# iesl/anncur

Hardware: AMD Instinct MI355X
Metric: queries/sec + Top-k-Recall@100 vs exact, CUR-256 on QxI score matrix (higher is better)
Workload: dtype bf16; 1 GPU; cfg2: Q=10000/GPU x I=100000 bf16 score matrix, 256 anchor items, 512 anchor queries, k=100, k_retvr=100; step = gather C_q + fused S_hat/top-k + exact top-k scan + overlap/recall; Q_per_gpu=10000, I=100000, anchors=256, anchor_queries=512, k=100, k_retvr=100

## Files before the change

### anncur_amd/csrc/common.hpp

```cpp
#pragma once
#include <hip/hip_runtime.h>
#include <stdint.h>
#include <stdarg.h>
#include <stdio.h>
#include "anncur_hip.h"

void anncur_set_error(const char *fmt, ...);
constexpr int LADDER_LEVELS = 8;
int anncur_internal_kth_value(const float *G, int64_t Q, int n, int64_t ldg, int k, float *out, int64_t out_stride, hipStream_t st, int coarse = 0,
							  float *ladder = nullptr, int k2 = 1, float *tau2 = nullptr);
int anncur_internal_approx_error_acc(const void *X, int x_dtype, int64_t ldx, const void *Et, int e_dtype, int64_t lde, const void *Aex, int a_dtype,
									 int64_t lda, int64_t Q, int64_t I, int64_t K, float *err_sq, float *norm_sq, void *stream);

int anncur_ensure_dyn_lds(const void *fn, int bytes);
int anncur_num_cu();
int anncur_event_pool(hipEvent_t **out, int n);
int anncur_internal_scan_rows_in_flight(int dtype);

#define ANNCUR_REQUIRE(cond, code, ...)                 \
	do {                                                \
		if (!(cond)) {                                  \
			anncur_set_error(__VA_ARGS__);              \
			return (code);                              \
		}                                               \
	} while (0)

#define ANNCUR_HIP_OK(expr)                                                              \
	do {                                                                                 \
		hipError_t e__ = (expr);                                                         \
		if (e__ != hipSuccess) {                                                         \
			anncur_set_error("%s failed: %s (%s:%d)", #expr, hipGetErrorString(e__), __FILE__, __LINE__); \
			return ANNCUR_E_HIP;                                                         \
		}                                                                                \
// ... 81 lines not shown
```

### anncur_amd/csrc/score16.hpp

```cpp
#pragma once

typedef __attribute__((ext_vector_type(4))) float f32x4;

template <int KP, int NW = 4>
struct Fused16Cfg {
	static constexpr int WAVES = NW;
	static constexpr int KS32 = KP / 32;
	static constexpr int K = KP / 16;
	static constexpr int CPR = KP / 8;
	static constexpr int TILE_BYTES = TILE_I * KP * 2;
	static constexpr int QCAP = 1024;
	static constexpr int DRAIN_AT = 192;
	static constexpr int QUEUE_OFF = 2 * TILE_BYTES;
	static constexpr int CNT_OFF = QUEUE_OFF + NW * QCAP * 8;
	static constexpr int TICKET_OFF = CNT_OFF + NW * 64 * 4;
	static constexpr int PIECES = TILE_BYTES / 1024 / NW;
	static_assert(PIECES >= 1, "a tile holds at least one 1 KB piece per wave");
	static constexpr int LVL_OFF = TICKET_OFF + 16;
	static constexpr int LCNT_OFF = LVL_OFF + NW * 64 * 4 * LADDER_LEVELS;
	static constexpr int JCUR_OFF = LCNT_OFF + NW * 64 * 16;
	static constexpr int LDS_BYTES = JCUR_OFF + NW * 64 * 4;
	static_assert(NW != 4 || LDS_BYTES <= 80 * 1024, "two workgroups per CU");
	static_assert(LADDER_LEVELS == 8, "two 128-bit reads per query; eight 16-bit fields in four counter words");
	static constexpr int BQ = 64 * NW;
// ... 158 lines not shown
		lds_wait_frag(ring[g % AR], after < DIST ? after : DIST);
		const bf16x8 a = __builtin_bit_cast(bf16x8, ring[g % AR]);
		const int s = g % K, ks = s >> 1, ih = s & 1;
		if (g < K) {
			accA[ih][0] = __builtin_amdgcn_mfma_f32_16x16x32_bf16(a, xb[0][ks], accA[ih][0], 0, 0, 0);
			accA[ih][1] = __builtin_amdgcn_mfma_f32_16x16x32_bf16(a, xb[1][ks], accA[ih][1], 0, 0, 0);
#pragma unroll
			for (int e = (g == 1 ? 0 : g) * EPS; e < (g == 0 ? 0 : g + 1) * EPS; ++e) F16_ELEM(accP, e, 2, tau_prev, item0_prev);
		} else {
			accB[ih][0] = __builtin_amdgcn_mfma_f32_16x16x32_bf16(a, xb[2][ks], accB[ih][0], 0, 0, 0);
			accB[ih][1] = __builtin_amdgcn_mfma_f32_16x16x32_bf16(a, xb[3][ks], accB[ih][1], 0, 0, 0);
#pragma unroll
			for (int e = (g - K == 1 ? 0 : g - K) * EPS; e < (g == K ? 0 : g - K + 1) * EPS; ++e) F16_ELEM(accA, e, 0, tau, item0);
		}
	}
#pragma unroll
	for (int ih = 0; ih < 2; ++ih)
#pragma unroll
		for (int q = 0; q < 2; ++q) accP[ih][q] = accB[ih][q];
#undef F16_READ
}

#define S16_SLICED (p.sliced)
template <int KP, int NW = 4>
__global__ __launch_bounds__(64 * NW, 2) void score16_kernel(const FusedParams p) {
	using C = Fused16Cfg<KP, NW>;
	constexpr int K = C::K, KS32 = C::KS32, CPR = C::CPR;
	extern __shared__ __attribute__((aligned(16))) unsigned char smem[];
	const int tid = threadIdx.x, lane = tid & 63, wave = tid >> 6;
	const int c16 = lane & 15, g4 = lane >> 4;
	const int wid = xcd_remap(blockIdx.x, p.n_wg);
	const int n_rb = (int)((p.Q + C::BQ - 1) / C::BQ);
	const int split = wid / n_rb, rb = wid - split * n_rb;

	bf16x8 xb[4][KS32];
	int64_t qv[4];
#pragma unroll
	for (int t = 0; t < 4; ++t) {
		qv[t] = (int64_t)rb * C::BQ + wave * 64 + 16 * t + c16;
		const bool ok = qv[t] < p.Q;
		const u32x4 *src = reinterpret_cast<const u32x4 *>(p.X + (ok ? qv[t] : 0) * p.ldx) + g4;
#pragma unroll
		for (int s = 0; s < KS32; ++s) {
			const u32x4 zero = {0u, 0u, 0u, 0u};
			const u32x4 w = ok ? src[4 * s] : zero;
			xb[t][s] = __builtin_bit_cast(bf16x8, w);
// ... 44 lines not shown
	const bool dyn = p.chunk_tiles > 0;
	uint32_t ticket_slot = lds_addr(smem + C::TICKET_OFF);
	uint32_t *const ctr_rb = p.chunk_ctr + (S16_SLICED ? (size_t)rb * N_SLICES : (size_t)rb);
	int slice = S16_SLICED ? xcc_id() : 0, tried = 0;
	if (dyn) {
		if (tid == 0) {
			uint32_t c0, c1;
			if (S16_SLICED) {
				c0 = slice_resolve(atomicAdd(ctr_rb + slice, 1u), ctr_rb, p.n_chunks, p.chunks_per_slice, slice, tried);
				c1 = c0 < (uint32_t)p.n_chunks ? slice_resolve(atomicAdd(ctr_rb + slice, 1u), ctr_rb, p.n_chunks, p.chunks_per_slice, slice, tried) : (uint32_t)p.n_chunks;
			} else {
				c0 = atomicAdd(ctr_rb, 2u); c1 = c0 + 1u;
			}
			if (p.chunk_owner) {
				if (c0 < (uint32_t)p.n_chunks) p.chunk_owner[(int64_t)rb * p.n_chunks + c0] = (uint8_t)split;
				if (c1 < (uint32_t)p.n_chunks) p.chunk_owner[(int64_t)rb * p.n_chunks + c1] = (uint8_t)split;
			}
			lds_write_u32(ticket_slot + 8u, c0);
			lds_write_u32(ticket_slot + 12u, c1);
			__builtin_amdgcn_s_waitcnt(0xC07F);
		}
		__syncthreads();
		const uint32_t c = lds_load_u32_uniform(ticket_slot + 8u), c1 = lds_load_u32_uniform(ticket_slot + 12u);
		t_cur = c < (uint32_t)p.n_chunks ? p.tile_begin + (int)c * p.chunk_tiles : -1;
		t_cend = min(t_cur + p.chunk_tiles, p.tile_end);
		t_next_chunk = c1 < (uint32_t)p.n_chunks ? p.tile_begin + (int)c1 * p.chunk_tiles : -1;
	}
	uint32_t dma_off[C::PIECES];
#pragma unroll
	for (int i = 0; i < C::PIECES; ++i) {
		const int pch = (wave_u * C::PIECES + i) * 64 + lane;
		const int row = pch / CPR, cs = pch % CPR;
		dma_off[i] = (uint32_t)(row * CPR + swz<CPR>(row, cs)) * 16u;
	}
	auto tile_dma_w = [&](int tile, uint32_t lds_buf) {
		const unsigned char *src = reinterpret_cast<const unsigned char *>(p.Et) + (int64_t)tile * C::TILE_BYTES;
#if defined(__HIP_DEVICE_COMPILE__)
#pragma unroll
		for (int i = 0; i < C::PIECES; ++i) {
			const uint32_t m0v = lds_buf + (uint32_t)(wave_u * C::PIECES + i) * 1024u;
			asm volatile("s_mov_b32 m0, %0\n\ts_nop 0\n\tglobal_load_lds_dwordx4 %1, %2" ::"s"(m0v), "v"(dma_off[i]), "s"(src) : "memory", "m0");
		}
#endif
	};
	if (t_cur >= 0) tile_dma_w(t_cur, lds_base);
	__builtin_amdgcn_s_waitcnt(0x0F70);
	__syncthreads();

	f32x4 accP[2][2];
// ... 11 lines not shown
	float tau_hi[2] = {tau[2], tau[3]};
#define R16_DRAIN_CHECK(J) do { if (fill >= w.base + C::DRAIN_AT * 8u) wq_drain<true>(w, fill); } while (0)
#define LADDER_STEP()                                                                                                           \
	do {                                                                                                                        \
		if (p.ladder_on) {                                                                                                      \
			const uint32_t ll_ = opaque_u32((uint32_t)lane);    \
			if (lad_pending) {                                                                                                  \
				ladder_refresh(lcnt_land + ll_ * 16u, w.lvl + ll_ * 32u, w.jcur + ll_ * 4u, p.ladder_k, (int)(ll_ & 15u), tau);     \
				tau_hi[0] = tau[2]; tau_hi[1] = tau[3];                                                                         \
				tau_prev[0] = fmaxf(tau_prev[0], tau[2]); tau_prev[1] = fmaxf(tau_prev[1], tau[3]);                             \
				lad_pending = false;                                                                                            \
			}                                                                                                                   \
			if ((++lad_tick & p.ladder_mask) == 0u) {                                                                           \
				ladder_fetch(w.lcnt, lcnt_land, (int)ll_);                                                                      \
				lad_pending = true;                                                                                             \
			}                                                                                                                   \
		}                                                                                                                       \
	} while (0)
#define STAGGER16_STEP(CUR)                                                                                                     \
	do {                                                                                                                        \
		const int J = t_cur;                                                                                                    \
		if (ticket_pending) {                                                                                                   \
			const uint32_t c = lds_load_u32_uniform(ticket_slot);                                                               \
			t_next_chunk = c < (uint32_t)p.n_chunks ? p.tile_begin + (int)c * p.chunk_tiles : -1;                               \
			ticket_pending = false;                                                                                             \
			ticket_slot ^= 4u;                                                                                                  \
		}                                                                                                                       \
		int nx = J + 1;                                                                                                         \
		bool crossed = false;                                                                                                   \
		if (nx >= t_cend) { nx = t_next_chunk; crossed = dyn && nx >= 0; }                                                      \
		if (nx >= 0) tile_dma_w(nx, lds_base + ((CUR) ^ 1) * C::TILE_BYTES);                                                    \
		uint32_t ticket = 0;                                                                                                    \
		if (crossed && tid == 0) ticket_draw(ticket, ctr_rb + slice);                                                           \
		LADDER_STEP();                                                                                                          \
		R16_DRAIN_CHECK(J);                                                                                                     \
		const uint32_t item0 = ((uint32_t)J * TILE_I + 4 * g4) | lane_code;                                                     \
		stagger16_tile<KP, CUR>(aoff, xb, accP, tau, tau_prev, item0, item0_prev, w, fill);                                        \
		tau_prev[0] = tau_hi[0]; tau_prev[1] = tau_hi[1]; item0_prev = item0;                                                   \
		ticket_wait(ticket);                                                                                                    \
		if (crossed) {                                                                                                          \
			if (tid == 0) {                                                                                                     \
				if (S16_SLICED) ticket = slice_resolve(ticket, ctr_rb, p.n_chunks, p.chunks_per_slice, slice, tried);             \
				lds_write_u32(ticket_slot, ticket);                                                                             \
				if (p.chunk_owner && ticket < (uint32_t)p.n_chunks) p.chunk_owner[(int64_t)rb * p.n_chunks + ticket] = (uint8_t)split; \
				__builtin_amdgcn_s_waitcnt(0xC07F);                                                                             \
			}                                                                                                                   \
			ticket_pending = true;                                                                                              \
			t_cend = min(nx + p.chunk_tiles, p.tile_end);                                                                       \
		}                                                                                                                       \
		__syncthreads();                                                                                                        \
		t_cur = nx;                                                                                                             \
	} while (0)
	ANNCUR_PAD_HERE();
	while (t_cur >= 0) {
		STAGGER16_STEP(0);
		if (t_cur < 0) break;
		STAGGER16_STEP(1);
	}
#undef STAGGER16_STEP
#undef LADDER_STEP
	wq_drain<true>(w, fill);
#define F16_LAST(e)                                                                                                             \
	filter16_one(accP[(e) >> 3][((e) >> 2) & 1][(e) & 3],                                                                       \
				 (uint32_t)((((e) >> 3) * 16 + ((e) & 3)) | ((uint32_t)(2 + (((e) >> 2) & 1)) << (WQ_ITEM_BITS + 4))),         \
				 tau_prev[((e) >> 2) & 1], item0_prev, w, fill)
	F16_LAST(0); F16_LAST(1); F16_LAST(2); F16_LAST(3); F16_LAST(4); F16_LAST(5); F16_LAST(6); F16_LAST(7);
	F16_LAST(8); F16_LAST(9); F16_LAST(10); F16_LAST(11); F16_LAST(12); F16_LAST(13); F16_LAST(14); F16_LAST(15);
#undef F16_LAST
#undef F16_ELEM
	wq_drain<true>(w, fill);
	if (p.ladder_on) {
		const int le = (int)opaque_u32((uint32_t)lane);
// ... 25 lines not shown
```

### anncur_amd/csrc/score_fused.hip

```cpp
#include <stdlib.h>
#include <math.h>
#include <type_traits>
#ifdef ANNCUR_PLACEMENT_PAD
#define ANNCUR_PAD_HERE() asm volatile(".rept %0\n\ts_nop 0\n\t.endr" ::"n"(ANNCUR_PLACEMENT_PAD) : "memory")
#else
#define ANNCUR_PAD_HERE() do { } while (0)
#endif
#include "select.hpp"
#include "wave_select.hpp"
#include "select_stream.hpp"

using namespace anncur;

namespace {

typedef __attribute__((ext_vector_type(8))) __bf16 bf16x8;
typedef __attribute__((ext_vector_type(16))) float f32x16;
typedef __attribute__((ext_vector_type(4))) unsigned int u32x4;

constexpr int TILE_I = 32;
constexpr int CHUNK_TILES = 4;

template <int KP, int QTV = ((KP <= 256) ? 2 : 1)>
struct FusedCfg {
// ... 18 lines not shown
}

struct FusedParams {
	const uint16_t *X; int64_t ldx;
	const uint16_t *Et;
	int64_t Q, I;
	int n_tiles, n_full_tiles;
	int S, tiles_per_split;
	int tile_begin, tile_end;
	int tile_step;
	int carry;
	int n_st, S0, st_per_split;
	int sample_leading;
	float *gmax; int n_groups;
	const float *tau; int tau_stride;
	uint2 *cand; uint32_t *seg_cnt; int capg;
	int nseg;
	int flush_tiles;
	int n_wg;
	int chunk_tiles, n_chunks;
	uint32_t *chunk_ctr;
	uint8_t *chunk_owner;
	int sliced, chunks_per_slice;
	int ladder_on; uint32_t ladder_k, ladder_mask;
	const float *ladder; uint32_t *ladder_cnt; float *tau_final;
	uint32_t *nfb;
	uint32_t zero_bytes;
};

__device__ __forceinline__ int xcd_remap(int b, int n) {
	const int q = n >> 3, r = n & 7, x = b & 7, l = b >> 3;
	return (x < r ? x * (q + 1) : r * (q + 1) + (x - r) * q) + l;
}

__device__ __forceinline__ void zero_ws_header(const FusedParams &p) {
	typedef __attribute__((ext_vector_type(4))) unsigned int zvec;
	zvec *const dst = reinterpret_cast<zvec *>(p.nfb);
	const uint32_t n = p.zero_bytes >> 4;
	for (uint32_t i = blockIdx.x * blockDim.x + threadIdx.x; i < n; i += gridDim.x * blockDim.x) dst[i] = (zvec){0u, 0u, 0u, 0u};
}


template <int KP>
__device__ __forceinline__ void tile_dma(const uint16_t *__restrict__ Et, int tile, unsigned char *buf, int wave, int lane) {
	constexpr int CPR = FusedCfg<KP>::CPR;
	constexpr int PER_WAVE = FusedCfg<KP>::TILE_BYTES / 1024 / 4;
	const unsigned char *src = reinterpret_cast<const unsigned char *>(Et + (int64_t)tile * TILE_I * KP);
#pragma unroll
	for (int i = 0; i < PER_WAVE; ++i) {
		const int piece = wave * PER_WAVE + i;
		const int pch = piece * 64 + lane;
// ... 812 lines not shown
		 \
		 \
		asm volatile("" ::: "memory");                                                                                          \
		__builtin_amdgcn_s_barrier();                                                                                           \
		asm volatile("" ::: "memory");                                                                                          \
	} while (0)
	for (int j = j_begin; j < j_end; j += 2) {
		ERR_STEP(0, j);
		if (j + 1 < j_end) ERR_STEP(1, j + 1);
	}
#undef ERR_STEP
#pragma unroll
	for (int t = 0; t < QT; ++t)
		if (qv[t] < p.Q) {
			atomicAdd(&err_sq[qv[t]], se[t]);
			atomicAdd(&norm_sq[qv[t]], sn[t]);
		}
}

#include "score_evalf.hpp"

struct SweepStages {
	int n, begin[3], end[3], tps[3], stride;
	int chunk, bq, n_chunks[3];
	const uint8_t *owner[3];
};

template <int KMAX>
__global__ __launch_bounds__(SEL_THREADS) void select_candidates_kernel(
	const uint2 *__restrict__ cand, const uint32_t *__restrict__ seg_cnt, int nseg, int S, SweepStages stg, int capg,
	const uint16_t *__restrict__ X, int64_t ldx, const uint16_t *__restrict__ Et, int64_t I, int KP, uint32_t k,
	float *__restrict__ out_val, int32_t *__restrict__ out_idx, uint32_t *__restrict__ n_fallback,
	const int32_t *__restrict__ hard_list, const uint32_t *__restrict__ hard_cnt, const float *__restrict__ tau_in, int tau_stride,
	const int32_t *__restrict__ remap) {
	extern __shared__ __attribute__((aligned(16))) unsigned char smem[];
	const SelState s = sel_carve<KMAX>(smem);
	float *xq = reinterpret_cast<float *>(smem + SelCfg<KMAX>::LDS_BYTES);
	uint32_t *bad = reinterpret_cast<uint32_t *>(xq + KP);
	const int tid = threadIdx.x, lane = tid & 63, wave = tid >> 6;
	auto score_of = [&](int64_t i) {
		float v = 0.f;
		const uint4 *er = reinterpret_cast<const uint4 *>(Et + i * KP);
		for (int c = 0; c < KP / 8; ++c) {
			const uint4 w = er[c];
			const uint32_t ww[4] = {w.x, w.y, w.z, w.w};
#pragma unroll
			for (int d = 0; d < 4; ++d) {
// ... 38 lines not shown
			for (uint32_t e0 = 0; e0 < maxc; e0 += WAVE) {
				const uint32_t e = e0 + lane;
				const bool in = e < c;
				const uint2 ce = in ? sp_ptr[e] : make_uint2(0, 0);
				sel_offer(s, in, __uint_as_float(ce.x), ce.y, tau, tau_key);
				sel_maybe_compact<KMAX>(s, k, tau, tau_key);
			}
		}
	}
	if (repair || full) {
		if (tid == 0) atomicAdd(n_fallback, 1u);
		for (int c = tid; c < KP; c += SEL_THREADS) xq[c] = bf16_bits_to_f32(X[q * ldx + c]);
		__syncthreads();
	}
	if (repair) {
		for (int sp = 0; sp < S; ++sp) {
			if (!((bad[sp >> 5] >> (sp & 31)) & 1u)) continue;
			for (int g = 0; g < stg.n; ++g) {
				if (stg.chunk > 0) {
					const uint8_t *own = stg.owner[g] + (q / stg.bq) * (int64_t)stg.n_chunks[g];
					int it = 0;
					for (int c = 0; c < stg.n_chunks[g]; ++c) {
						if (own[c] != (uint8_t)sp) continue;
						const int64_t i_beg = (int64_t)(stg.begin[g] + c * stg.chunk) * TILE_I;
						const int64_t i_end = (int64_t)min(stg.begin[g] + (c + 1) * stg.chunk, stg.end[g]) * TILE_I;
						for (int64_t i0 = i_beg; i0 < i_end; i0 += SEL_THREADS, ++it) {
							const int64_t i = i0 + tid;
							const bool in = i < i_end && i < I;
							const float v = in ? score_of(i) : 0.f;
							sel_offer(s, in, v, (uint32_t)i, tau, tau_key);
							if ((it & 15) == 15) sel_maybe_compact<KMAX>(s, k, tau, tau_key);
						}
					}
					sel_maybe_compact<KMAX>(s, k, tau, tau_key);
					continue;
				}
				if (stg.stride > 1) {
					int it = 0;
					for (int tb = stg.begin[g] + sp; tb < stg.end[g]; tb += 8 * stg.stride, ++it) {
						const int tile = tb + (tid >> 5) * stg.stride;
						const int64_t i = (int64_t)tile * TILE_I + (tid & 31);
						const bool in = tile < stg.end[g] && i < I;
						const float v = in ? score_of(i) : 0.f;
						sel_offer(s, in, v, (uint32_t)i, tau, tau_key);
						if ((it & 15) == 15) sel_maybe_compact<KMAX>(s, k, tau, tau_key);
					}
					sel_maybe_compact<KMAX>(s, k, tau, tau_key);
					continue;
// ... 138 lines not shown
	wsel_finish<0, 4, WqCfg<KW>::E, true>(w, k, out_val + q * (int64_t)k, out_idx + q * (int64_t)k, remap);
}

}
namespace {
#include "score_wide.hpp"
}
namespace {

struct FusedPlan {
	bool ok;
	bool wide;
	int QT, BQ, n_rb, n_tiles, n_full, S, tiles_per_split, group, n_st, S0, st_per_split, n_groups, capg, kmax, flush_tiles;
	int n_stages, stage_end[3], stage_tps[3], stage_flush[3], stage_pred[3];
	int leading;
	int lg;
	int nseg;
	bool body16;
	bool bodyef;
	bool bodyq16;
	int chunk;
	bool ladder;
	int ladder_k2;
	size_t off_lcnt, off_lvl, off_tau2;
	size_t off_gmax, off_tval, off_tidx, off_segcnt, off_cand, off_tau, off_hard, off_ctr, off_owner, total;
};

int num_cu() { return anncur_num_cu(); }

size_t align256(size_t x) { return (x + 255) & ~(size_t)255; }
int next_pow2(int x) { int p = 1; while (p < x) p <<= 1; return p; }

void plan_stages(FusedPlan &P, int64_t Q, int k, double exp_hits, bool staged, double fmin, int unit_items) {
	double frac[3] = {1.0, 1.0, 1.0};
	P.n_stages = 1;
	if (staged) {
		const double H0 = exp_hits, c_hit = 2.4e-11 * (double)Q;
		const double c_stage = k <= WSEL_K ? 25e-6 + 3e-9 * (double)Q : (k <= WQ_K2 ? 25e-6 + 1.2e-8 * (double)Q : 25e-6 + 1.4e-11 * (double)Q * 0.3 * H0);
		auto later = [&](double f) { const double h = 1.2 * k / f; return h < H0 ? h : H0; };
		double best = H0 * c_hit;
		static const double grid[] = {0.02, 0.03, 0.04, 0.06, 0.08, 0.10, 0.12, 0.15, 0.18, 0.22, 0.26, 0.30, 0.35, 0.40, 0.50};
		const int ng = (int)(sizeof(grid) / sizeof(grid[0]));
		for (int i = 0; i < ng; ++i) {
			const double f1 = grid[i];
			if (f1 < fmin) continue;
			const double c2 = (f1 * H0 + (1 - f1) * later(f1)) * c_hit + c_stage;
// ... 106 lines not shown
	if (S > 255) S = P.chunk > 0 ? 255 : (S > 256 ? 256 : S);
	if (S > P.n_tiles) S = P.n_tiles;
	P.tiles_per_split = (P.n_tiles + S - 1) / S;
	P.S = (P.n_tiles + P.tiles_per_split - 1) / P.tiles_per_split;
	constexpr int64_t LADDER_WAVE_SLACK = (int64_t)(LADDER_PERIOD + 2) * TILE_I + Fused16Cfg<256>::DRAIN_AT;
	const bool ladder_fits = I < 65536 || (int64_t)k + (int64_t)P.S * LADDER_WAVE_SLACK <= 32768;
	const bool ladder_possible = !no_ladder && ticketed && P.n_groups <= 4096 && ladder_fits;
	P.body16 = can16 && !mfma32 && !evalf && (mfma16 || k <= (ladder_possible ? BODY16_MAX_K_LADDER : BODY16_MAX_K));
	plan_prepass_splits(P, slots);
	P.lg = (P.body16 || P.bodyq16 || P.bodyef) ? 1 : 2;
	const double exp_hits = plan_segments(P, k, leading);
	const double per_lane_tile = exp_hits / ((double)P.n_tiles * 2.0);
	int ft = (int)(0.35 / (per_lane_tile > 1e-9 ? per_lane_tile : 1e-9));
	P.flush_tiles = ft < 1 ? 1 : (ft > 8 ? 8 : ft);
	P.ladder = P.body16 && ladder_possible;
	{
		double r = (double)k * ((double)P.n_st * TILE_I / (double)I) * (leading ? 2.0 : 1.25);
		int k2 = (int)(r + 0.5);
		if (k2 > k / 2) k2 = k / 2;
		if (k2 < 3) k2 = 3;
		if (k2 > k) k2 = k;
		P.ladder_k2 = k2;
	}
	plan_stages(P, Q, k, exp_hits, !P.ladder && (k <= WQ_K2 ? P.nseg <= WAVE : true) && P.n_tiles >= 24 * P.S, 4.0 * P.S / P.n_tiles, TILE_I);
	plan_workspace(P, Q, k, (size_t)P.n_rb * 3 * 4 * N_SLICES, (size_t)3 * P.n_rb * (size_t)(P.n_tiles / (P.chunk > 0 ? P.chunk : P.n_tiles) + 2));
	return P;
}

int launch_tau_refine(const uint2 *cand, const uint32_t *seg_cnt, int nseg, int capg, int64_t Q, int k, int kmax, float *tau, int tau_stride,
					  int prefilter, hipStream_t st) {
	int rc;
	if (k <= WQ_K2 && nseg <= WAVE) {
		if (k <= WSEL_K) {
			constexpr int lds = 4 * WaveSelLayout<WqCfg<128>::CAP>::BYTES;
			if ((rc = anncur_ensure_dyn_lds((const void *)select_wave_kernel<true, 128>, lds)) != ANNCUR_OK) return rc;
			hipLaunchKernelGGL((select_wave_kernel<true, 128>), dim3((unsigned)ceil_div64(Q, 4)), dim3(256), lds, st, cand, seg_cnt, nseg, capg, Q,
							   (uint32_t)k, (float *)nullptr, (int32_t *)nullptr, (uint32_t *)nullptr, (int32_t *)nullptr, tau, tau_stride, prefilter, (const int32_t *)nullptr);
		} else {
			constexpr int lds = 4 * StreamSelLayout::BYTES;
			hipLaunchKernelGGL((select_stream_kernel<true, 2>), dim3((unsigned)ceil_div64(Q, 4)), dim3(256), lds, st, cand, seg_cnt, nseg, capg, Q,
							   (uint32_t)k, (float *)nullptr, (int32_t *)nullptr, (uint32_t *)nullptr, (int32_t *)nullptr, tau, tau_stride, prefilter, (const int32_t *)nullptr);
		}
	} else {
#define LAUNCH_TAU(KM)                                                                                                        \
		do {                                                                                                                  \
			if ((rc = anncur_ensure_dyn_lds((const void *)tau_block_kernel<KM>, (int)SelCfg<KM>::LDS_BYTES)) != ANNCUR_OK) return rc; \
// ... 37 lines not shown
			constexpr int lds = 4 * StreamSelLayout::BYTES;                                                                       \
			hipLaunchKernelGGL((select_stream_kernel<false, EE>), dim3((unsigned)ceil_div64(Q, 4)), dim3(256), lds, st, cand, seg_cnt, P.nseg, P.capg, Q, \
							   (uint32_t)k, out_val, out_idx, hc, hl, const_cast<float *>(tau), tau_stride, (P.n_stages > 1 || P.ladder) ? 1 : 0, remap); \
		} while (0)
		if (k <= WSEL_K) LAUNCH_WSEL(128);
		else if (k <= 256) LAUNCH_SSEL(4);
		else if (k <= 512) LAUNCH_SSEL(8);
		else LAUNCH_SSEL(16);
#undef LAUNCH_SSEL
#undef LAUNCH_WSEL
		ANNCUR_LAUNCH_OK();
		hard_list = hl; hard_cnt = hc;
		sel_grid = (unsigned)(Q < 1024 ? Q : 1024);
	}
	if (P.kmax == 128) LAUNCH_SELECT(128); else if (P.kmax == 512) LAUNCH_SELECT(512); else LAUNCH_SELECT(2048);
#undef LAUNCH_SELECT
	ANNCUR_LAUNCH_OK();
	return ANNCUR_OK;
}

int launch_threshold(const FusedPlan &P, const float *gmax, int64_t Q, int k, unsigned char *ws, const float *&tau, int &tau_stride, hipStream_t st) {
	if (P.n_groups <= 4096) {
		float *t = (float *)(ws + P.off_tau);
		const int rc = P.ladder ? anncur_internal_kth_value(gmax, Q, P.n_groups, P.n_groups, k, t, 1, st, 1, (float *)(ws + P.off_lvl), P.ladder_k2, (float *)(ws + P.off_tau2))
								: anncur_internal_kth_value(gmax, Q, P.n_groups, P.n_groups, k, t, 1, st, 1);
		tau = t; tau_stride = 1;
		return rc;
	}
	float *tval = (float *)(ws + P.off_tval);
	tau = tval + (k - 1); tau_stride = k;
	return anncur_rowwise_topk(gmax, ANNCUR_F32, Q, P.n_groups, P.n_groups, k, tval, (int32_t *)(ws + P.off_tidx), st);
}


struct CoScan {
	hipStream_t aux;
	hipEvent_t *ev;
	const void *A; int a_dtype; int64_t lda, Q, I; int32_t k;
	float *val; int32_t *idx;
	int slots, next;
	int64_t row_end[8];
};

int co_plan(CoScan &co, int slots) {
	if (slots > 8) slots = 8;
	if (slots < 1) slots = 1;
	const int64_t round = anncur_internal_scan_rows_in_flight(co.a_dtype);
// ... 98 lines not shown
	return ANNCUR_OK;
#undef EV
}

template <int KP, int QTV = FusedCfg<KP>::QT>
int launch_fused(const FusedPlan &P, const TopkCall &c) {
	using Cfg = FusedCfg<KP, QTV>;
	unsigned char *const ws = c.ws; const hipStream_t st = c.st; const EvalArgs *const ea = c.ea;
	FusedParams p{};
	p.X = (const uint16_t *)c.X; p.ldx = c.ldx; p.Et = (const uint16_t *)c.Et; p.Q = c.Q; p.I = c.I;
	p.n_tiles = P.n_tiles; p.n_full_tiles = P.n_full; p.S = P.S; p.tiles_per_split = P.tiles_per_split;
	p.tile_begin = 0; p.tile_end = P.n_tiles; p.carry = 0; p.tile_step = 1;
	p.n_st = P.n_st; p.S0 = P.S0; p.st_per_split = P.st_per_split; p.sample_leading = P.leading;
	p.gmax = (float *)(ws + P.off_gmax); p.n_groups = P.n_groups;
	p.cand = (uint2 *)(ws + P.off_cand); p.seg_cnt = (uint32_t *)(ws + P.off_segcnt); p.capg = P.capg; p.flush_tiles = P.flush_tiles;
	p.nfb = (uint32_t *)ws; p.nseg = P.nseg;
	p.ladder_on = P.ladder ? 1 : 0; p.ladder_k = (uint32_t)c.k; p.ladder_mask = (uint32_t)(LADDER_PERIOD - 1);
	p.ladder = (const float *)(ws + P.off_lvl); p.ladder_cnt = (uint32_t *)(ws + P.off_lcnt); p.tau_final = (float *)(ws + P.off_tau2);

	const int chunk = (P.chunk > 0 && (Cfg::QT == 2 || P.bodyq16)) ? P.chunk : 0;
	const int owner_stride = P.n_rb * (P.n_tiles / (chunk > 0 ? chunk : P.n_tiles) + 2);
	const int tile_step = (!P.body16 && !P.bodyq16 && !P.bodyef && P.S > 1 && chunk == 0) ? P.S : 1;
	SweepStages stages{};
	stages.stride = tile_step; stages.chunk = chunk; stages.bq = P.BQ;
	for (int g = 0, prev = 0; g < P.n_stages; prev = P.stage_end[g], ++g) {
		stages.n_chunks[g] = chunk > 0 ? (P.stage_end[g] - prev + chunk - 1) / chunk : 0;
		stages.owner[g] = (const uint8_t *)(ws + P.off_owner) + (size_t)g * owner_stride;
	}

	auto launch_prepass = [&]() -> int {
		p.n_wg = P.n_rb * P.S0;
		FusedParams pp = p;
		pp.zero_bytes = (uint32_t)((chunk > 0 || P.ladder) ? P.off_gmax : 256);
		if (ea && ea->Et_hint) { pp.Et = ea->Et_hint; pp.sample_leading = 1; }
		if constexpr (KP <= 256 && QTV == 2) {
			if (P.body16 && P.group == 16) {
				if (const int rcl = anncur_ensure_dyn_lds((const void *)prepass16_kernel<KP>, Prepass16Cfg<KP>::LDS_BYTES)) return rcl;
				hipLaunchKernelGGL((prepass16_kernel<KP>), dim3(p.n_wg), dim3(256), Prepass16Cfg<KP>::LDS_BYTES, st, pp);
				return ANNCUR_OK;
			}
		}
		if (P.group == 16)
			hipLaunchKernelGGL((score_prepass_kernel<KP, 16, QTV>), dim3(p.n_wg), dim3(256), 2 * Cfg::TILE_BYTES, st, pp);
		else
			hipLaunchKernelGGL((score_prepass_kernel<KP, 4, QTV>), dim3(p.n_wg), dim3(256), 2 * Cfg::TILE_BYTES, st, pp);
		return ANNCUR_OK;
	};
	auto launch_stage = [&](int stg, int prev) -> int {
		p.n_wg = P.n_rb * P.S;
		p.tile_begin = prev; p.tile_end = P.stage_end[stg]; p.tiles_per_split = P.stage_tps[stg];
		p.flush_tiles = P.stage_flush[stg]; p.carry = stg > 0;
		p.tile_step = tile_step;
		if (chunk > 0) {
			p.chunk_tiles = chunk; p.n_chunks = (p.tile_end - p.tile_begin + chunk - 1) / chunk;
			p.sliced = P.bodyq16 ? 1 : 0;
			p.chunks_per_slice = (p.n_chunks + N_SLICES - 1) / N_SLICES;
			p.chunk_ctr = (uint32_t *)(ws + P.off_ctr) + (size_t)stg * P.n_rb * N_SLICES;
			p.chunk_owner = (uint8_t *)(ws + P.off_owner) + (size_t)stg * owner_stride;
		}
		auto launch = [&](auto kernel, int lds, auto... more) -> int {
			if (const int rcl = anncur_ensure_dyn_lds((const void *)kernel, lds)) return rcl;
			hipLaunchKernelGGL(kernel, dim3(p.n_wg), dim3(256), lds, st, p, more...);
			return ANNCUR_OK;
		};
		if constexpr (KP <= 256 && QTV == 2) {
			if (P.bodyef && !ea) { anncur_set_error("launch_fused: evalf plan without the exact matrix"); return ANNCUR_E_INVALID; }
			if (P.bodyef) return launch(evalf_kernel<KP>, EvalFCfg<KP>::LDS_BYTES, ea->A, ea->lda, ea->err_sq, ea->norm_sq);
		}
		if constexpr (KP == 512) {
			if (P.bodyq16) return launch(scoreq16_kernel<KP>, FusedQ16Cfg<KP>::LDS_BYTES);
		}
		if constexpr (KP <= 256 && QTV == 2) {
			if (P.body16) return launch(score16_kernel<KP>, Fused16Cfg<KP>::LDS_BYTES);
		}
		if constexpr (Cfg::QT == 2) {
			if (P.stage_pred[stg]) return launch(score_sweep_kernel<KP, true, QTV>, Cfg::LDS_BYTES);
		}
		return launch(score_sweep_kernel<KP, false, QTV>, Cfg::LDS_BYTES);
	};
	return run_pipeline(P, c, stages, 1, p.tau, p.tau_stride, launch_prepass, launch_stage);
}
// ... 379 lines not shown
```

### anncur_amd/csrc/topk.hip

```cpp
#include <stdlib.h>
#include <atomic>
#include "select.hpp"
#include "wave_select.hpp"

using namespace anncur;

namespace {

constexpr int SCAN_PASS = 2048;

template <typename T> struct VecOf;
template <> struct VecOf<float> { static constexpr int N = 4; };
template <> struct VecOf<uint16_t> { static constexpr int N = 8; };

typedef uint32_t u32x4 __attribute__((ext_vector_type(4)));

template <typename T>
__device__ __forceinline__ float vec_elem(const u32x4 &r, int e);
template <>
__device__ __forceinline__ float vec_elem<float>(const u32x4 &r, int e) { return __uint_as_float(r[e]); }
template <>
__device__ __forceinline__ float vec_elem<uint16_t>(const u32x4 &r, int e) {
	const uint32_t w = r[e >> 1];
	return __uint_as_float((e & 1) ? (w & 0xffff0000u) : (w << 16));
// ... 416 lines not shown
				else {
					if ((x >> 24) == bin0) atomicAdd(&w.hist[(x >> 16) & 255u], 1u);
					else if ((x >> 24) == binG0) atomicAdd(&hist2[(x >> 16) & 255u], 1u);
				}
			}
		}
		__builtin_amdgcn_wave_barrier();
		if (pass == 0) {
			wsel_find_bin(w.hist, lane, k, bin0, a0, hb);
			wsel_find_bin(w.hist, lane, k2, binG0, aG0, hb);
		} else {
			uint32_t bin1, a1, binG1 = 0;
			wsel_find_bin(w.hist, lane, k - a0, bin1, a1, hb);
			T = ((bin0 << 8) | bin1) << 16;
			wsel_find_bin(binG0 == bin0 ? w.hist : hist2, lane, k2 - aG0, binG1, a1, hb);
			G = ((binG0 << 8) | binG1) << 16;
		}
		__builtin_amdgcn_wave_barrier();
	}
}

__global__ __launch_bounds__(256) void kth_value_wave_kernel(const float *__restrict__ G, int64_t Q, int n, int64_t ldg, uint32_t k,
															  float *__restrict__ out, int64_t out_stride, int n_pad, int coarse,
															  float *__restrict__ ladder, uint32_t k2, float *__restrict__ tau2) {
	extern __shared__ __attribute__((aligned(16))) unsigned char kth_smem[];
	const uint32_t lane = (uint32_t)lane_id();
	const int wave = threadIdx.x >> 6;
	uint32_t *hist = reinterpret_cast<uint32_t *>(kth_smem) + wave * (256 + n_pad + (ladder ? 256 : 0));
	uint32_t *keys = hist + 256;
	const int64_t q = (int64_t)blockIdx.x * 4 + wave;
	if (q >= Q) return;
	const float *g = G + q * ldg;
	for (uint32_t j = lane; j < (uint32_t)n; j += WAVE) {
		const float v = g[j];
		keys[j] = (v == v) ? f32_sortable(v) : 0u;
	}
	__builtin_amdgcn_wave_barrier();
	WaveSel w;
	w.whi = keys; w.wlo = nullptr; w.sort_buf = nullptr; w.hist = hist;
	w.cnt = (uint32_t)n; w.tau_hi = 0; w.tau_lo = 0; w.tau = 0.f;
	uint32_t need;
	uint32_t kk, gk = 0;
	if (ladder) kth2_coarse(w, hist + 256 + n_pad, w.whi, (uint32_t)n, k, k2 < k ? k2 : k, kk, gk);
	else if (coarse) kk = wsel_kth<false, 2>(w, w.whi, (uint32_t)n, k, need, w.whi, 0u);
	else kk = wsel_kth<false, 4>(w, w.whi, (uint32_t)n, k, need, w.whi, 0u);
	if (lane == 0) out[q * out_stride] = f32_unsortable(kk);
	if (ladder) {
		const float t0 = f32_unsortable(kk), g = f32_unsortable(gk);
		float d = g - t0;
		if (!(d > 0.f) || !(d < INFINITY)) d = 0.f;
		if (lane < (uint32_t)LADDER_LEVELS) ladder[q * LADDER_LEVELS + lane] = t0 + d * ((float)(lane + 1) * (1.0f / LADDER_LEVELS));
		if (lane == 0 && tau2) tau2[q] = t0;
	}
}

template <typename T, int KMAX>
__global__ __launch_bounds__(SEL_THREADS) void rerank_kernel(const T *__restrict__ A, int64_t I, int64_t lda,
															  const int32_t *__restrict__ approx_idx, int64_t ld_idx,
															  uint32_t k_retvr, uint32_t k_out, float *__restrict__ out_val,
															  int32_t *__restrict__ out_idx) {
	extern __shared__ __attribute__((aligned(16))) unsigned char smem[];
	const SelState s = sel_carve<KMAX>(smem);
	sel_init(s);
	const int tid = threadIdx.x;
	const int64_t q = blockIdx.x;
	const T *row = A + q * lda;
	const int32_t *ai = approx_idx + q * ld_idx;
	float tau = -INFINITY;
	uint64_t tau_key = 0;
	for (uint32_t j0 = 0; j0 < k_retvr; j0 += SEL_THREADS) {
		const uint32_t j = j0 + tid;
		int32_t it = (j < k_retvr) ? ai[j] : -1;
		const bool in = it >= 0 && (int64_t)it < I;
		const float v = in ? load_as_f32<T>(row + it) : 0.f;
		sel_offer(s, in, v, (uint32_t)it, tau, tau_key);
// ... 122 lines not shown
	if (c < n_cols) dst[r * ldd + c] = cvt<TS, TD>(src[r * lds_ + c]);
}

__global__ __launch_bounds__(256) void copy_bytes_kernel(const uint4 *__restrict__ src, uint4 *__restrict__ dst, size_t n16,
														  const unsigned char *__restrict__ src_tail, unsigned char *__restrict__ dst_tail, int n_tail) {
	const size_t i = (size_t)blockIdx.x * 256 + threadIdx.x;
	if (i < n16) dst[i] = src[i];
	if (blockIdx.x == 0 && (int)threadIdx.x < n_tail) dst_tail[threadIdx.x] = src_tail[threadIdx.x];
}

template <typename F>
int dispatch2(int sd, int dd, F &&f) {
	if (sd == ANNCUR_F32 && dd == ANNCUR_F32) return f((const float *)nullptr, (float *)nullptr);
	if (sd == ANNCUR_F32 && dd == ANNCUR_BF16) return f((const float *)nullptr, (uint16_t *)nullptr);
	if (sd == ANNCUR_BF16 && dd == ANNCUR_F32) return f((const uint16_t *)nullptr, (float *)nullptr);
	return f((const uint16_t *)nullptr, (uint16_t *)nullptr);
}

int kmax_class(int k) { return k <= 128 ? 128 : (k <= 512 ? 512 : 2048); }

}

int anncur_internal_kth_value(const float *G, int64_t Q, int n, int64_t ldg, int k, float *out, int64_t out_stride, hipStream_t st, int coarse,
							  float *ladder, int k2, float *tau2) {
	ANNCUR_REQUIRE(n >= 1 && n <= KTH_MAX_N && k >= 1 && k <= n, ANNCUR_E_INVALID, "kth_value: need 1 <= k <= n <= 4096");
	const unsigned grid = (unsigned)ceil_div64(Q, 4);
	const int n_pad = (n + 63) & ~63;
	const int lds = 4 * (256 + n_pad + (ladder ? 256 : 0)) * 4;
	int rc;
	if (lds > 64 * 1024 && (rc = anncur_ensure_dyn_lds((const void *)kth_value_wave_kernel, lds)) != ANNCUR_OK) return rc;
	hipLaunchKernelGGL(kth_value_wave_kernel, dim3(grid), dim3(256), lds, st, G, Q, n, ldg, (uint32_t)k, out, out_stride, n_pad, coarse, ladder, (uint32_t)(k2 < 1 ? 1 : k2), tau2);
	ANNCUR_LAUNCH_OK();
	return ANNCUR_OK;
}

int anncur_internal_scan_rows_in_flight(int dtype) {
	constexpr int MAX_DEV = 64;
	static std::atomic<int> cached[MAX_DEV][2];
	int dev = 0;
	if (hipGetDevice(&dev) != hipSuccess) { (void)hipGetLastError(); dev = 0; }
	const int di = dtype == ANNCUR_F32 ? 0 : 1;
	std::atomic<int> *slot = (dev >= 0 && dev < MAX_DEV) ? &cached[dev][di] : nullptr;
	int v = slot ? slot->load(std::memory_order_relaxed) : 0;
	if (v == 0) {
		int occ = 0;
		const size_t lds = 4 * (size_t)WaveSelLayout<WS_CAP>::BYTES;
		const hipError_t e = di == 0 ? hipOccupancyMaxActiveBlocksPerMultiprocessor(&occ, rowwise_topk_wave_kernel<float>, 256, lds)
									 : hipOccupancyMaxActiveBlocksPerMultiprocessor(&occ, rowwise_topk_wave_kernel<uint16_t>, 256, lds);
		if (e != hipSuccess || occ < 1) { (void)hipGetLastError(); occ = 3; }
		v = occ * 4 * anncur_num_cu();
		if (slot) slot->store(v, std::memory_order_relaxed);
	}
	return v;
}
// ... 246 lines not shown
```

Baseline: 12.57 million queries/s.

## Pre-seed ladder counters from sampled gmax and rotate chunk order past sample region

```diff
diff --git a/anncur_amd/csrc/common.hpp b/anncur_amd/csrc/common.hpp
--- a/anncur_amd/csrc/common.hpp
+++ b/anncur_amd/csrc/common.hpp
@@ -8,7 +8,7 @@
 void anncur_set_error(const char *fmt, ...);
 constexpr int LADDER_LEVELS = 8;
 int anncur_internal_kth_value(const float *G, int64_t Q, int n, int64_t ldg, int k, float *out, int64_t out_stride, hipStream_t st, int coarse = 0,
-							  float *ladder = nullptr, int k2 = 1, float *tau2 = nullptr);
+							  float *ladder = nullptr, int k2 = 1, float *tau2 = nullptr, uint32_t *ladder_cnt = nullptr);
 int anncur_internal_approx_error_acc(const void *X, int x_dtype, int64_t ldx, const void *Et, int e_dtype, int64_t lde, const void *Aex, int a_dtype,
 									 int64_t lda, int64_t Q, int64_t I, int64_t K, float *err_sq, float *norm_sq, void *stream);
 
diff --git a/anncur_amd/csrc/score16.hpp b/anncur_amd/csrc/score16.hpp
--- a/anncur_amd/csrc/score16.hpp
+++ b/anncur_amd/csrc/score16.hpp
@@ -204,6 +204,7 @@
 }
 
 #define S16_SLICED (p.sliced)
+#define S16_CHUNK_TILE(c) (p.tile_begin + chunk_pos((int)(c), p.chunk_rot, p.n_chunks) * p.chunk_tiles)
 template <int KP, int NW = 4>
 __global__ __launch_bounds__(64 * NW, 2) void score16_kernel(const FusedParams p) {
 	using C = Fused16Cfg<KP, NW>;
@@ -294,9 +295,10 @@
 		}
 		__syncthreads();
 		const uint32_t c = lds_load_u32_uniform(ticket_slot + 8u), c1 = lds_load_u32_uniform(ticket_slot + 12u);
-		t_cur = c < (uint32_t)p.n_chunks ? p.tile_begin + (int)c * p.chunk_tiles : -1;
+		t_cur = c < (uint32_t)p.n_chunks ? S16_CHUNK_TILE(c) : -1;
 		t_cend = min(t_cur + p.chunk_tiles, p.tile_end);
-		t_next_chunk = c1 < (uint32_t)p.n_chunks ? p.tile_begin + (int)c1 * p.chunk_tiles : -1;
+		t_next_chunk = c1 < (uint32_t)p.n_chunks ? S16_CHUNK_TILE(c1) : -1;
+		if (t_cur >= 0 && t_cur < p.sample_end) w.lad_on = 0u;
 	}
 	uint32_t dma_off[C::PIECES];
 #pragma unroll
@@ -354,8 +356,8 @@
 		const int J = t_cur;                                                                                                    \
 		if (ticket_pending) {                                                                                                   \
 			const uint32_t c = lds_load_u32_uniform(ticket_slot);                                                               \
-			t_next_chunk = c < (uint32_t)p.n_chunks ? p.tile_begin + (int)c * p.chunk_tiles : -1;                               \
-			ticket_pending = false;                                                                                             \
+			t_next_chunk = c < (uint32_t)p.n_chunks ? S16_CHUNK_TILE(c) : -1;                                                   \
+			ticket_pending = false;                                                                                          \
 			ticket_slot ^= 4u;                                                                                                  \
 		}                                                                                                                       \
 		int nx = J + 1;                                                                                                         \
@@ -379,7 +381,9 @@
 			}                                                                                                                   \
 			ticket_pending = true;                                                                                              \
 			t_cend = min(nx + p.chunk_tiles, p.tile_end);                                                                       \
-		}                                                                                                                       \
+			 \
+			if (w.lad_on && nx < p.sample_end) { wq_drain<true>(w, fill); w.lad_on = 0u; }                                      \
+		}                                                                                                                \
 		__syncthreads();                                                                                                        \
 		t_cur = nx;                                                                                                             \
 	} while (0)
diff --git a/anncur_amd/csrc/score_fused.hip b/anncur_amd/csrc/score_fused.hip
--- a/anncur_amd/csrc/score_fused.hip
+++ b/anncur_amd/csrc/score_fused.hip
@@ -64,11 +64,14 @@
 	uint32_t *chunk_ctr;
 	uint8_t *chunk_owner;
 	int sliced, chunks_per_slice;
+	int chunk_rot, sample_end;
 	int ladder_on; uint32_t ladder_k, ladder_mask;
 	const float *ladder; uint32_t *ladder_cnt; float *tau_final;
 	uint32_t *nfb;
 	uint32_t zero_bytes;
 };
+
+__host__ __device__ __forceinline__ constexpr int chunk_pos(int c, int rot, int n_chunks) { return c + rot >= n_chunks ? c + rot - n_chunks : c + rot; }
 
 __device__ __forceinline__ int xcd_remap(int b, int n) {
 	const int q = n >> 3, r = n & 7, x = b & 7, l = b >> 3;
@@ -927,7 +930,7 @@
 
 struct SweepStages {
 	int n, begin[3], end[3], tps[3], stride;
-	int chunk, bq, n_chunks[3];
+	int chunk, bq, n_chunks[3], rot;
 	const uint8_t *owner[3];
 };
 
@@ -1012,8 +1015,9 @@
 					int it = 0;
 					for (int c = 0; c < stg.n_chunks[g]; ++c) {
 						if (own[c] != (uint8_t)sp) continue;
-						const int64_t i_beg = (int64_t)(stg.begin[g] + c * stg.chunk) * TILE_I;
-						const int64_t i_end = (int64_t)min(stg.begin[g] + (c + 1) * stg.chunk, stg.end[g]) * TILE_I;
+						const int cp = chunk_pos(c, stg.rot, stg.n_chunks[g]);
+						const int64_t i_beg = (int64_t)(stg.begin[g] + cp * stg.chunk) * TILE_I;
+						const int64_t i_end = (int64_t)min(stg.begin[g] + (cp + 1) * stg.chunk, stg.end[g]) * TILE_I;
 						for (int64_t i0 = i_beg; i0 < i_end; i0 += SEL_THREADS, ++it) {
 							const int64_t i = i0 + tid;
 							const bool in = i < i_end && i < I;
@@ -1198,6 +1202,7 @@
 	int chunk;
 	bool ladder;
 	int ladder_k2;
+	int sample_last;
 	size_t off_lcnt, off_lvl, off_tau2;
 	size_t off_gmax, off_tval, off_tidx, off_segcnt, off_cand, off_tau, off_hard, off_ctr, off_owner, total;
 };
@@ -1350,6 +1355,11 @@
 		if (k2 > k) k2 = k;
 		P.ladder_k2 = k2;
 	}
+	P.sample_last = 0;
+	if (P.ladder && leading && P.group == 16 && P.chunk > 0) {
+		const int r = (P.n_st + P.chunk - 1) / P.chunk, n_chunks = (P.n_tiles + P.chunk - 1) / P.chunk;
+		if (r < n_chunks) P.sample_last = r;
+	}
 	plan_stages(P, Q, k, exp_hits, !P.ladder && (k <= WQ_K2 ? P.nseg <= WAVE : true) && P.n_tiles >= 24 * P.S, 4.0 * P.S / P.n_tiles, TILE_I);
 	plan_workspace(P, Q, k, (size_t)P.n_rb * 3 * 4 * N_SLICES, (size_t)3 * P.n_rb * (size_t)(P.n_tiles / (P.chunk > 0 ? P.chunk : P.n_tiles) + 2));
 	return P;
@@ -1433,7 +1443,8 @@
 int launch_threshold(const FusedPlan &P, const float *gmax, int64_t Q, int k, unsigned char *ws, const float *&tau, int &tau_stride, hipStream_t st) {
 	if (P.n_groups <= 4096) {
 		float *t = (float *)(ws + P.off_tau);
-		const int rc = P.ladder ? anncur_internal_kth_value(gmax, Q, P.n_groups, P.n_groups, k, t, 1, st, 1, (float *)(ws + P.off_lvl), P.ladder_k2, (float *)(ws + P.off_tau2))
+		const int rc = P.ladder ? anncur_internal_kth_value(gmax, Q, P.n_groups, P.n_groups, k, t, 1, st, 1, (float *)(ws + P.off_lvl), P.ladder_k2, (float *)(ws + P.off_tau2),
+														 P.sample_last > 0 ? (uint32_t *)(ws + P.off_lcnt) : (uint32_t *)nullptr)
 								: anncur_internal_kth_value(gmax, Q, P.n_groups, P.n_groups, k, t, 1, st, 1);
 		tau = t; tau_stride = 1;
 		return rc;
@@ -1578,7 +1589,7 @@
 	const int owner_stride = P.n_rb * (P.n_tiles / (chunk > 0 ? chunk : P.n_tiles) + 2);
 	const int tile_step = (!P.body16 && !P.bodyq16 && !P.bodyef && P.S > 1 && chunk == 0) ? P.S : 1;
 	SweepStages stages{};
-	stages.stride = tile_step; stages.chunk = chunk; stages.bq = P.BQ;
+	stages.stride = tile_step; stages.chunk = chunk; stages.bq = P.BQ; stages.rot = chunk > 0 ? P.sample_last : 0;
 	for (int g = 0, prev = 0; g < P.n_stages; prev = P.stage_end[g], ++g) {
 		stages.n_chunks[g] = chunk > 0 ? (P.stage_end[g] - prev + chunk - 1) / chunk : 0;
 		stages.owner[g] = (const uint8_t *)(ws + P.off_owner) + (size_t)g * owner_stride;
@@ -1613,6 +1624,7 @@
 			p.chunks_per_slice = (p.n_chunks + N_SLICES - 1) / N_SLICES;
 			p.chunk_ctr = (uint32_t *)(ws + P.off_ctr) + (size_t)stg * P.n_rb * N_SLICES;
 			p.chunk_owner = (uint8_t *)(ws + P.off_owner) + (size_t)stg * owner_stride;
+			p.chunk_rot = P.sample_last; p.sample_end = P.sample_last * chunk < p.tile_end ? P.sample_last * chunk : p.tile_end;
 		}
 		auto launch = [&](auto kernel, int lds, auto... more) -> int {
 			if (const int rcl = anncur_ensure_dyn_lds((const void *)kernel, lds)) return rcl;
diff --git a/anncur_amd/csrc/topk.hip b/anncur_amd/csrc/topk.hip
--- a/anncur_amd/csrc/topk.hip
+++ b/anncur_amd/csrc/topk.hip
@@ -462,7 +462,7 @@
 
 __global__ __launch_bounds__(256) void kth_value_wave_kernel(const float *__restrict__ G, int64_t Q, int n, int64_t ldg, uint32_t k,
 															  float *__restrict__ out, int64_t out_stride, int n_pad, int coarse,
-															  float *__restrict__ ladder, uint32_t k2, float *__restrict__ tau2) {
+															  float *__restrict__ ladder, uint32_t k2, float *__restrict__ tau2, uint32_t *__restrict__ ladder_cnt) {
 	extern __shared__ __attribute__((aligned(16))) unsigned char kth_smem[];
 	const uint32_t lane = (uint32_t)lane_id();
 	const int wave = threadIdx.x >> 6;
@@ -489,8 +489,32 @@
 		const float t0 = f32_unsortable(kk), g = f32_unsortable(gk);
 		float d = g - t0;
 		if (!(d > 0.f) || !(d < INFINITY)) d = 0.f;
-		if (lane < (uint32_t)LADDER_LEVELS) ladder[q * LADDER_LEVELS + lane] = t0 + d * ((float)(lane + 1) * (1.0f / LADDER_LEVELS));
+		const float lvl = t0 + d * ((float)((lane & (LADDER_LEVELS - 1)) + 1) * (1.0f / LADDER_LEVELS));
+		if (lane < (uint32_t)LADDER_LEVELS) ladder[q * LADDER_LEVELS + lane] = lvl;
 		if (lane == 0 && tau2) tau2[q] = t0;
+		if (ladder_cnt) {
+			uint32_t lk[LADDER_LEVELS], ge[LADDER_LEVELS];
+#pragma unroll
+			for (int j = 0; j < LADDER_LEVELS; ++j) {
+				const float lj = __uint_as_float((uint32_t)__builtin_amdgcn_readlane((int)__float_as_uint(lvl), j));
+				lk[j] = (lj == lj) ? f32_sortable(lj) : 0xffffffffu;
+				ge[j] = 0u;
+			}
+			for (uint32_t j0 = 0; j0 < (uint32_t)n; j0 += WAVE) {
+				const uint32_t j = j0 + lane, key = j < (uint32_t)n ? keys[j] : 0u;
+#pragma unroll
+				for (int i = 0; i < LADDER_LEVELS; ++i) ge[i] += (uint32_t)__builtin_popcountll(__ballot(key >= lk[i]));
+			}
+			if (lane < (uint32_t)(LADDER_LEVELS / 2)) {
+				uint32_t word = 0;
+#pragma unroll
+				for (int i = 0; i < LADDER_LEVELS / 2; ++i) {
+					const uint32_t a = ge[2 * i] - ge[2 * i + 1], b = 2 * i + 2 < LADDER_LEVELS ? ge[2 * i + 1] - ge[2 * i + 2] : ge[2 * i + 1];
+					word = lane == (uint32_t)i ? ((a < k ? a : k) | ((b < k ? b : k) << 16)) : word;
+				}
+				ladder_cnt[q * (LADDER_LEVELS / 2) + lane] = word;
+			}
+		}
 	}
 }
 
@@ -659,14 +683,15 @@
 }
 
 int anncur_internal_kth_value(const float *G, int64_t Q, int n, int64_t ldg, int k, float *out, int64_t out_stride, hipStream_t st, int coarse,
-							  float *ladder, int k2, float *tau2) {
+							  float *ladder, int k2, float *tau2, uint32_t *ladder_cnt) {
 	ANNCUR_REQUIRE(n >= 1 && n <= KTH_MAX_N && k >= 1 && k <= n, ANNCUR_E_INVALID, "kth_value: need 1 <= k <= n <= 4096");
 	const unsigned grid = (unsigned)ceil_div64(Q, 4);
 	const int n_pad = (n + 63) & ~63;
 	const int lds = 4 * (256 + n_pad + (ladder ? 256 : 0)) * 4;
 	int rc;
 	if (lds > 64 * 1024 && (rc = anncur_ensure_dyn_lds((const void *)kth_value_wave_kernel, lds)) != ANNCUR_OK) return rc;
-	hipLaunchKernelGGL(kth_value_wave_kernel, dim3(grid), dim3(256), lds, st, G, Q, n, ldg, (uint32_t)k, out, out_stride, n_pad, coarse, ladder, (uint32_t)(k2 < 1 ? 1 : k2), tau2);
+	hipLaunchKernelGGL(kth_value_wave_kernel, dim3(grid), dim3(256), lds, st, G, Q, n, ldg, (uint32_t)k, out, out_stride, n_pad, coarse, ladder, (uint32_t)(k2 < 1 ? 1 : k2), tau2,
+					   ladder ? ladder_cnt : (uint32_t *)nullptr);
 	ANNCUR_LAUNCH_OK();
 	return ANNCUR_OK;
 }
```

Result: faster. 12.83 million queries/s (median of 6 runs) (+2.1%).
